# foollh/PicoPose

Hardware: AMD Instinct MI355X
Metric: image-crops/sec (224x224, 162 templates) (higher is better)
Workload: dtype f32 tensors; networks: f32 operands split into 2 f16 terms (22 bits) on f16 MFMA with f32 accumulate; stage-1 contraction: f16 MFMA operands, f32 accumulate, exact f32 re-evaluation of near-ties; PnP f64

## Files before the change

### picopose_amd/csrc/pp_attn.hip

```cpp

#include <hip/hip_runtime.h>
#include <stdint.h>
#include <stdlib.h>
#include "../../include/picopose_hip.h"
#include "pp_common.h"

namespace {

typedef float f32x16 __attribute__((ext_vector_type(16)));
typedef float f4 __attribute__((ext_vector_type(4)));

constexpr int HD = 64, KC = 32, KLD = 68;

constexpr int KTAIL_MAX = 4;
template <int WPB>
__global__ __launch_bounds__(64 * WPB) void attn_kernel(const float* __restrict__ qkv, int T, int heads, float scale,
                                                        float* __restrict__ out, _Float16* __restrict__ out_hl) {
    __shared__ __attribute__((aligned(16))) float Ks[KC * KLD];
    __shared__ __attribute__((aligned(16))) float Vs[KC * HD];
    const int tid = threadIdx.x, lane = tid & 63, w = tid >> 6, l31 = lane & 31, lh = lane >> 5;
    const int b = blockIdx.y / heads, h = blockIdx.y % heads;
    const int C3 = 3 * heads * HD;
    const float* base = qkv + (size_t)b * T * C3 + h * HD;
    const int q = blockIdx.x * (32 * WPB) + w * 32 + l31;
    const int qc = q < T ? q : T - 1;

    float qr[32];
    {
        const float* qp = base + (size_t)qc * C3 + 32 * lh;
#pragma unroll
        for (int p = 0; p < 32; p += 4) {
            const f4 v = *(const f4*)(qp + p);
            const float sc2 = scale * 1.44269504088896340736f;
            qr[p] = v.x * sc2; qr[p + 1] = v.y * sc2; qr[p + 2] = v.z * sc2; qr[p + 3] = v.w * sc2;
        }
    }
    f32x16 o0, o1;
#pragma unroll
    for (int e = 0; e < 16; ++e) o0[e] = o1[e] = 0.f;
    float mrun = -INFINITY, lrun = 0.f;

    const float* kp = base + heads * HD;
    const float* vp = base + 2 * heads * HD;
    const int ktail = (T % KC) <= KTAIL_MAX ? T % KC : 0;
    const int kend = T - ktail;
    for (int k0 = 0; k0 < kend; k0 += KC) {
        __syncthreads();
#pragma unroll
        for (int idx = tid; idx < KC * HD / 4; idx += 64 * WPB) {
            const int row = idx >> 4, c4 = (idx & 15) * 4;
            f4 kv = {0.f, 0.f, 0.f, 0.f}, vv = {0.f, 0.f, 0.f, 0.f};
            if (k0 + row < T) {
                kv = *(const f4*)(kp + (size_t)(k0 + row) * C3 + c4);
                vv = *(const f4*)(vp + (size_t)(k0 + row) * C3 + c4);
            }
            *(f4*)(Ks + row * KLD + c4) = kv;
            *(f4*)(Vs + row * HD + c4) = vv;
        }
        __syncthreads();
        f32x16 s;
#pragma unroll
        for (int e = 0; e < 16; ++e) s[e] = 0.f;
#pragma unroll
        for (int p4 = 0; p4 < 32; p4 += 4) {
            const f4 kf = *(const f4*)(Ks + l31 * KLD + 32 * lh + p4);
            s = __builtin_amdgcn_mfma_f32_32x32x2f32(kf.x, qr[p4], s, 0, 0, 0);
            s = __builtin_amdgcn_mfma_f32_32x32x2f32(kf.y, qr[p4 + 1], s, 0, 0, 0);
            s = __builtin_amdgcn_mfma_f32_32x32x2f32(kf.z, qr[p4 + 2], s, 0, 0, 0);
            s = __builtin_amdgcn_mfma_f32_32x32x2f32(kf.w, qr[p4 + 3], s, 0, 0, 0);
        }
        float mx = -INFINITY;
        if (k0 + KC <= T) {
#pragma unroll
            for (int e = 0; e < 16; ++e) mx = fmaxf(mx, s[e]);
        } else {
#pragma unroll
            for (int e = 0; e < 16; ++e) {
                const int key = k0 + (e & 3) + 8 * (e >> 2) + 4 * lh;
                s[e] = key < T ? s[e] : -INFINITY;
                mx = fmaxf(mx, s[e]);
            }
        }
        mx = fmaxf(mx, __shfl_xor(mx, 32));
        const float mnew = fmaxf(mrun, mx);
        const float alpha = __builtin_amdgcn_exp2f(mrun - mnew);
        float ls = 0.f;
#pragma unroll
        for (int e = 0; e < 16; ++e) {
            s[e] = __builtin_amdgcn_exp2f(s[e] - mnew);
            ls += s[e];
        }
        ls += __shfl_xor(ls, 32);
        lrun = lrun * alpha + ls;
        mrun = mnew;
#pragma unroll
        for (int e = 0; e < 16; ++e) {
            o0[e] *= alpha;
            o1[e] *= alpha;
        }
#pragma unroll
        for (int e = 0; e < 16; ++e) {
            const int key = (e & 3) + 8 * (e >> 2) + 4 * lh;
            const float v0 = Vs[key * HD + l31], v1 = Vs[key * HD + 32 + l31];
            o0 = __builtin_amdgcn_mfma_f32_32x32x2f32(v0, s[e], o0, 0, 0, 0);
            o1 = __builtin_amdgcn_mfma_f32_32x32x2f32(v1, s[e], o1, 0, 0, 0);
        }
    }
    for (int kx = kend; kx < T; ++kx) {
        const float* kr = kp + (size_t)kx * C3 + 32 * lh;
        float sp = 0.f;
#pragma unroll
        for (int p = 0; p < 32; p += 4) {
            const f4 kf = *(const f4*)(kr + p);
            sp = fmaf(kf.x, qr[p], sp);
            sp = fmaf(kf.y, qr[p + 1], sp);
            sp = fmaf(kf.z, qr[p + 2], sp);
            sp = fmaf(kf.w, qr[p + 3], sp);
        }
        const float sc = sp + __shfl_xor(sp, 32);
        const float mnew = fmaxf(mrun, sc);
        const float alpha = __builtin_amdgcn_exp2f(mrun - mnew);
        const float pk = __builtin_amdgcn_exp2f(sc - mnew);
        lrun = lrun * alpha + pk;
        mrun = mnew;
        const float* vr = vp + (size_t)kx * C3 + 4 * lh;
#pragma unroll
        for (int g = 0; g < 4; ++g) {
            const f4 v0 = *(const f4*)(vr + 8 * g), v1 = *(const f4*)(vr + 32 + 8 * g);
            o0[4 * g] = fmaf(v0.x, pk, o0[4 * g] * alpha);
            o0[4 * g + 1] = fmaf(v0.y, pk, o0[4 * g + 1] * alpha);
            o0[4 * g + 2] = fmaf(v0.z, pk, o0[4 * g + 2] * alpha);
            o0[4 * g + 3] = fmaf(v0.w, pk, o0[4 * g + 3] * alpha);
            o1[4 * g] = fmaf(v1.x, pk, o1[4 * g] * alpha);
            o1[4 * g + 1] = fmaf(v1.y, pk, o1[4 * g + 1] * alpha);
            o1[4 * g + 2] = fmaf(v1.z, pk, o1[4 * g + 2] * alpha);
            o1[4 * g + 3] = fmaf(v1.w, pk, o1[4 * g + 3] * alpha);
        }
    }
    if (q < T) {
        const float inv = 1.0f / lrun;
        const size_t obase = ((size_t)b * T + q) * (heads * HD) + h * HD;
#pragma unroll
        for (int e = 0; e < 16; ++e) {
            const int d = (e & 3) + 8 * (e >> 2) + 4 * lh;
            const float a0 = o0[e] * inv, a1 = o1[e] * inv;
            if (out) {
                out[obase + d] = a0;
                out[obase + 32 + d] = a1;
            }
            if (out_hl) {
                _Float16 hh, ll;
                pp_split_f16_chk(a0, hh, ll);
                out_hl[2 * obase + pp_hl_col(d, 0)] = hh;
                out_hl[2 * obase + pp_hl_col(d, 1)] = ll;
                pp_split_f16_chk(a1, hh, ll);
                out_hl[2 * obase + pp_hl_col(32 + d, 0)] = hh;
                out_hl[2 * obase + pp_hl_col(32 + d, 1)] = ll;
            }
        }
    }
}

typedef _Float16 h8 __attribute__((ext_vector_type(8)));
constexpr int KHLD = 72;
constexpr int VLD = 96;
typedef _Float16 h4 __attribute__((ext_vector_type(4)));
typedef __fp16 fp16x4_t __attribute__((__vector_size__(4 * sizeof(__fp16))));
constexpr int OLD = 68;
constexpr float P_SCALE = 1024.f;

__device__ __forceinline__ int vt_slot(int key) {
    const int s = key >> 4, r = key & 15;
    return s * 16 + ((r >> 2) & 1) * 8 + (r & 3) + 4 * (r >> 3);
}

template <int TERMS>
struct RingGeom {
    static constexpr int ROWH = 64 * TERMS;
    static constexpr int CPR = ROWH / 8;
    static constexpr int RPP = 64 / CPR;
    static constexpr int NPT = KC / RPP;
    static constexpr int STAGE_H = 2 * KC * ROWH;
};

template <bool HLIN, int TERMS = 2, int RING = 0, int WPB = 0>
__global__ __launch_bounds__(WPB > 4 ? 64 * WPB : 256) __attribute__((amdgpu_waves_per_eu(3, 3))) void attn_f16x3_kernel(const void* __restrict__ qkv_any, int T, int heads, float scale,
                                                         float* __restrict__ out, _Float16* __restrict__ out_hl,
                                                         float* __restrict__ lse, int ntx, int npairs) {
    static_assert(RING == 0 || (HLIN && WPB >= 1 && (WPB <= 4 || (WPB == 9 && RING == 8))), "the LDS-DMA ring copies operand rows");
    constexpr bool RESIDENT = RING == 8 && WPB == 9;
    using RG = RingGeom<TERMS>;
    extern __shared__ __attribute__((aligned(16))) unsigned char smem[];
    _Float16* Kh = (_Float16*)smem;
    _Float16* Kl = Kh + KC * KHLD;
    _Float16* Vh = Kl + KC * KHLD;
    _Float16* Vl = Vh + KC * VLD;
    const int tid = threadIdx.x, nthr = blockDim.x, lane = tid & 63, w = RING ? __builtin_amdgcn_readfirstlane(tid >> 6) : tid >> 6, l31 = lane & 31, lh = lane >> 5;
    const int xcd = blockIdx.x & 7, jj = blockIdx.x >> 3, bx = jj % ntx, pair = (jj / ntx) * 8 + xcd;
    if (pair >= npairs) return;
    const int b = pair / heads, h = pair % heads;
    const int C3 = 3 * heads * HD;
    const float* base = (const float*)qkv_any + (size_t)b * T * C3 + h * HD;
    const _Float16* hbase = (const _Float16*)qkv_any + ((size_t)b * T * C3 + h * HD) * TERMS;
    const int q = (bx * (nthr >> 6) + w) * 32 + l31;
    const int qc = q < T ? q : T - 1;

    h8 qh[4], ql[4];
    if (HLIN) {
        const _Float16* qp = hbase + (size_t)qc * C3 * TERMS;
#pragma unroll
        for (int s = 0; s < 4; ++s) {
            qh[s] = *(const h8*)(qp + TERMS * (16 * s + 8 * lh));
            if (TERMS == 2) ql[s] = *(const h8*)(qp + 2 * (16 * s + 8 * lh) + 8);
            else ql[s] = h8{0, 0, 0, 0, 0, 0, 0, 0};
        }
    } else {
        const float* qp = base + (size_t)qc * C3;
#pragma unroll
        for (int s = 0; s < 4; ++s) {
            const f4 a = *(const f4*)(qp + 16 * s + 8 * lh), c = *(const f4*)(qp + 16 * s + 8 * lh + 4);
#pragma unroll
            for (int i = 0; i < 4; ++i) {
                _Float16 hh, ll;
                pp_split_f16_chk(a[i], hh, ll);
                qh[s][i] = hh;
                ql[s][i] = ll;
                pp_split_f16_chk(c[i], hh, ll);
                qh[s][4 + i] = hh;
                ql[s][4 + i] = ll;
            }
        }
    }
    f32x16 o0, o1;
#pragma unroll
    for (int e = 0; e < 16; ++e) o0[e] = o1[e] = 0.f;
    float mrun = -INFINITY, lrun = 0.f;
    const float* kp = base + heads * HD;
    const float* vp = base + 2 * heads * HD;
    const float S_DESCALE = scale * 1.44269504088896340736f / (PP_A_SCALE * PP_A_SCALE);
    constexpr float O_RESCALE = 1.0f / PP_A_SCALE;
#define SOFTMAX_STEP(K0)                                                                                          \
    float mx = -INFINITY;                                                                                         \
    if ((K0) + KC > Tm) {        \
        _Pragma("unroll") for (int e = 0; e < 16; ++e) {                                                          \
            const int key = (K0) + (e & 3) + 8 * (e >> 2) + 4 * lh;                                               \
            sacc[e] = key < Tm ? sacc[e] : -INFINITY;                                                             \
        }                                                                                                         \
    }                                                                                                             \
    _Pragma("unroll") for (int e = 0; e < 16; ++e) mx = fmaxf(mx, sacc[e]);                                       \
    mx = fmaxf(mx, __shfl_xor(mx, 32));                                                                           \
    const float mnew = fmaxf(mrun, mx * S_DESCALE);                                                               \
    const float alpha = __builtin_amdgcn_exp2f(mrun - mnew);                                                      \
    const float shift = 10.0f - mnew;                                                                             \
    float ls = 0.f;                                                                                               \
    h8 ph[2], pl[2];                                                                                              \
    _Pragma("unroll") for (int e = 0; e < 16; ++e) {                                                              \
        const float x = __builtin_amdgcn_exp2f(fmaf(sacc[e], S_DESCALE, shift));              \
        ls += x;                                                                                                  \
        const _Float16 hh = (_Float16)x;                                                                          \
        ph[e >> 3][e & 7] = hh;                                                                                   \
        pl[e >> 3][e & 7] = (_Float16)(x - (float)hh);                                                            \
    }                                                                                                             \
    ls += __shfl_xor(ls, 32);                                                                                     \
    lrun = lrun * alpha + ls;                                                                                     \
    mrun = mnew;                                                                                                  \
    if (__builtin_amdgcn_ballot_w64(alpha != 1.0f) != 0) {                                                        \
        _Pragma("unroll") for (int e = 0; e < 16; ++e) {                                                          \
            o0[e] *= alpha;                                                                                       \
            o1[e] *= alpha;                                                                                       \
        }                                                                                                         \
    }

    constexpr int TAILMAX = 4;
    const int ntail = (T % KC) <= TAILMAX ? T % KC : 0, Tm = T - ntail;
    constexpr int NIT = HLIN ? 2 : 4;
    h8 pk[HLIN ? 2 * NIT : 1], pv[HLIN ? 2 * NIT : 1];
    f4 fk[HLIN ? 1 : NIT], fv[HLIN ? 1 : NIT];
    auto fetch = [&](int k0) __attribute__((always_inline)) {
#pragma unroll
        for (int it = 0; it < NIT; ++it) {
            const int idx = tid + it * nthr;
            if (HLIN) {
                const int row = idx >> 3, g = idx & 7;
                h8 z = {0, 0, 0, 0, 0, 0, 0, 0};
                pk[2 * it] = pk[2 * it + 1] = pv[2 * it] = pv[2 * it + 1] = z;
                if (idx < KC * (HD / 8) && k0 + row < Tm) {
                    const _Float16* kp2 = hbase + ((size_t)(k0 + row) * C3 + heads * HD + 8 * g) * TERMS;
                    const _Float16* vp2 = hbase + ((size_t)(k0 + row) * C3 + 2 * heads * HD + 8 * g) * TERMS;
                    pk[2 * it] = *(const h8*)kp2;
                    pv[2 * it] = *(const h8*)vp2;
                    if (TERMS == 2) {
                        pk[2 * it + 1] = *(const h8*)(kp2 + 8);
                        pv[2 * it + 1] = *(const h8*)(vp2 + 8);
                    }
                }
            } else {
                const int row = idx >> 4, c4 = (idx & 15) * 4;
                fk[it] = fv[it] = f4{0.f, 0.f, 0.f, 0.f};
                if (idx < KC * (HD / 4) && k0 + row < Tm) {
                    fk[it] = *(const f4*)(kp + (size_t)(k0 + row) * C3 + c4);
                    fv[it] = *(const f4*)(vp + (size_t)(k0 + row) * C3 + c4);
                }
            }
        }
    };
    auto commit = [&]() __attribute__((always_inline)) {
#pragma unroll
        for (int it = 0; it < NIT; ++it) {
            const int idx = tid + it * nthr;
            if (HLIN) {
                if (idx >= KC * (HD / 8)) continue;
                const int row = idx >> 3, g = idx & 7, slot = vt_slot(row);
                *(h8*)(Kh + row * KHLD + 8 * g) = pk[2 * it];
                *(h8*)(Vh + slot * VLD + 8 * g) = pv[2 * it];
                if (TERMS == 2) {
                    *(h8*)(Kl + row * KHLD + 8 * g) = pk[2 * it + 1];
                    *(h8*)(Vl + slot * VLD + 8 * g) = pv[2 * it + 1];
                }
            } else {
                if (idx >= KC * (HD / 4)) continue;
                const int row = idx >> 4, c4 = (idx & 15) * 4, slot = vt_slot(row);
                h4 khh, kll, vhh, vll;
#pragma unroll
                for (int i = 0; i < 4; ++i) {
                    _Float16 hh, ll;
                    pp_split_f16_chk(fk[it][i], hh, ll);
                    khh[i] = hh;
                    kll[i] = ll;
                    pp_split_f16_chk(fv[it][i], hh, ll);
                    vhh[i] = hh;
                    vll[i] = ll;
                }
                *(h4*)(Kh + row * KHLD + c4) = khh;
                *(h4*)(Kl + row * KHLD + c4) = kll;
                *(h4*)(Vh + slot * VLD + c4) = vhh;
                *(h4*)(Vl + slot * VLD + c4) = vll;
            }
        }
    };
    constexpr int NPW = RING ? (2 * RG::NPT + (WPB > 0 ? WPB : 1) - 1) / (WPB > 0 ? WPB : 1) : 1;
    unsigned poff[NPW];
    int prow[NPW];
    const __amdgpu_buffer_rsrc_t Hr = __builtin_amdgcn_make_buffer_rsrc(
        (void*)hbase, 0, RING ? (int)(((size_t)(T - 1) * C3 + 2 * heads * HD + HD) * 2 * TERMS) : 0, 0x00020000);
    if (RING) {
#pragma unroll
        for (int i = 0; i < NPW; ++i) {
            const int p = (w + (WPB > 0 ? WPB : 1) * i) % (2 * RG::NPT), isv = p / RG::NPT;
            const int rho = (p % RG::NPT) * RG::RPP + lane / RG::CPR, pos = lane % RG::CPR;
            int key, xk;
            if (isv) {
                const int r16 = rho & 15;
                key = (rho & 16) | (((r16 >> 2) & 1) << 3) | ((r16 >> 3) << 2) | (r16 & 3);
                xk = TERMS == 2 ? ((rho & 1) | (((rho >> 1) & 1) << 3)) : (((rho >> 1) & 1) << 2);
            } else {
                key = rho;
                xk = TERMS == 2 ? (rho & 15) : ((rho >> 1) & 7);
            }
            prow[i] = key;
            poff[i] = (unsigned)(((size_t)key * C3 + (size_t)(1 + isv) * heads * HD) * 2 * TERMS + (unsigned)((pos ^ xk) * 16));
        }
    }
    auto ring_pieces = [&](int k0, int stage, int i0, int i1) __attribute__((always_inline)) {
        _Float16* st = (_Float16*)smem + stage * RG::STAGE_H;
        const unsigned kbytes = (unsigned)((size_t)k0 * C3 * 2 * TERMS);
#pragma unroll
        for (int i = 0; i < NPW; ++i) {
            if (i < i0 || i >= i1) continue;
            const int p = (w + (WPB > 0 ? WPB : 1) * i) % (2 * RG::NPT);
            const unsigned off = (k0 + prow[i] < Tm) ? poff[i] + kbytes : 0xFFFFFFFFu;
            __builtin_amdgcn_raw_ptr_buffer_load_lds(Hr, (__attribute__((address_space(3))) void*)(st + p * 512), 16, off, 0, 0, 0);
        }
    };
    auto ring_issue = [&](int k0, int stage) __attribute__((always_inline)) { ring_pieces(k0, stage, 0, NPW); };
    auto ring_slot = [&](int k0, int stage, int g) __attribute__((always_inline)) {
        if ((g * NPW) / 6 != ((g + 1) * NPW) / 6) {
            __builtin_amdgcn_sched_barrier(0);
            ring_pieces(k0, stage, (g * NPW) / 6, ((g + 1) * NPW) / 6);
            __builtin_amdgcn_sched_barrier(0);
        }
    };
    if constexpr (RING > 0) {
        const int nch = (Tm + KC - 1) / KC;
#pragma unroll
        for (int c = 0; c < (RESIDENT ? RING : RING - 1); ++c) ring_issue(c * KC, c);
        int stage = 0, fill = RING - 1;
        const int kx = TERMS == 2 ? (l31 & 15) : ((l31 >> 1) & 7);
        for (int c = 0; c < nch; ++c) {
            const int k0 = c * KC;
            if constexpr (RESIDENT) {
                switch (c) {
                    case 0: asm volatile("s_waitcnt vmcnt(%0)" ::"n"(7 * NPW) : "memory"); break;
                    case 1: asm volatile("s_waitcnt vmcnt(%0)" ::"n"(6 * NPW) : "memory"); break;
                    case 2: asm volatile("s_waitcnt vmcnt(%0)" ::"n"(5 * NPW) : "memory"); break;
                    case 3: asm volatile("s_waitcnt vmcnt(%0)" ::"n"(4 * NPW) : "memory"); break;
                    case 4: asm volatile("s_waitcnt vmcnt(%0)" ::"n"(3 * NPW) : "memory"); break;
                    case 5: asm volatile("s_waitcnt vmcnt(%0)" ::"n"(2 * NPW) : "memory"); break;
                    case 6: asm volatile("s_waitcnt vmcnt(%0)" ::"n"(1 * NPW) : "memory"); break;
                    default: asm volatile("s_waitcnt vmcnt(0)" ::: "memory"); break;
                }
            } else {
                asm volatile("s_waitcnt vmcnt(%0)" ::"n"((RING - 2) * NPW) : "memory");
            }
            __syncthreads();
#ifndef PP_ATTN_SPREAD
            if constexpr (!RESIDENT) ring_issue(k0 + (RING - 1) * KC, fill);
#endif
            const int kn = k0 + (RING - 1) * KC;
            (void)kn;
            const _Float16* Kst = (const _Float16*)smem + stage * RG::STAGE_H;
            const _Float16* Vst = Kst + KC * RG::ROWH;
            f32x16 sacc;
#pragma unroll
            for (int e = 0; e < 16; ++e) sacc[e] = 0.f;
#pragma unroll
            for (int s = 0; s < 4; ++s) {
                const int ch = TERMS == 2 ? 2 * (2 * s + lh) : 2 * s + lh;
                const h8 kh = *(const h8*)(Kst + l31 * RG::ROWH + ((ch ^ kx) * 8));
                if (TERMS == 2) {
                    const h8 kl = *(const h8*)(Kst + l31 * RG::ROWH + (((ch + 1) ^ kx) * 8));
                    sacc = __builtin_amdgcn_mfma_f32_32x32x16_f16(kl, qh[s], sacc, 0, 0, 0);
                    sacc = __builtin_amdgcn_mfma_f32_32x32x16_f16(kh, ql[s], sacc, 0, 0, 0);
                }
                sacc = __builtin_amdgcn_mfma_f32_32x32x16_f16(kh, qh[s], sacc, 0, 0, 0);
#ifdef PP_ATTN_SPREAD
                ring_slot(kn, fill, s);
#endif
            }
            SOFTMAX_STEP(k0)
            auto vfrag = [&](int term, int s, int dhalf) __attribute__((always_inline)) -> h8 {
                const int col = 32 * dhalf + 16 * ((lane >> 4) & 1) + 4 * (lane & 3);
                const int row = 16 * s + 8 * lh + ((lane & 15) >> 2);
                const int ch = TERMS == 2 ? 2 * (col >> 3) + term : (col >> 3);
                auto at = [&](int r) __attribute__((always_inline)) -> const _Float16* {
                    const int xv = TERMS == 2 ? ((r & 1) | (((r >> 1) & 1) << 3)) : (((r >> 1) & 1) << 2);
                    return Vst + r * RG::ROWH + ((ch ^ xv) * 8) + (col & 7);
                };
                const fp16x4_t lo4 = __builtin_amdgcn_ds_read_tr16_b64_v4f16((__attribute__((address_space(3))) fp16x4_t*)at(row));
                const fp16x4_t hi4 = __builtin_amdgcn_ds_read_tr16_b64_v4f16((__attribute__((address_space(3))) fp16x4_t*)at(row + 4));
                h8 r;
#pragma unroll
                for (int e = 0; e < 4; ++e) {
                    r[e] = (_Float16)lo4[e];
                    r[4 + e] = (_Float16)hi4[e];
                }
                return r;
            };
#pragma unroll
            for (int s = 0; s < 2; ++s) {
                const h8 v0h = vfrag(0, s, 0), v1h = vfrag(0, s, 1);
                if (TERMS == 2) {
                    const h8 v0l = vfrag(1, s, 0), v1l = vfrag(1, s, 1);
                    o0 = __builtin_amdgcn_mfma_f32_32x32x16_f16(v0l, ph[s], o0, 0, 0, 0);
                    o0 = __builtin_amdgcn_mfma_f32_32x32x16_f16(v0h, pl[s], o0, 0, 0, 0);
                    o1 = __builtin_amdgcn_mfma_f32_32x32x16_f16(v1l, ph[s], o1, 0, 0, 0);
                    o1 = __builtin_amdgcn_mfma_f32_32x32x16_f16(v1h, pl[s], o1, 0, 0, 0);
                }
                o0 = __builtin_amdgcn_mfma_f32_32x32x16_f16(v0h, ph[s], o0, 0, 0, 0);
                o1 = __builtin_amdgcn_mfma_f32_32x32x16_f16(v1h, ph[s], o1, 0, 0, 0);
#ifdef PP_ATTN_SPREAD
                ring_slot(kn, fill, 4 + s);
#endif
            }
            fill = stage;
            stage = stage + 1 == RING ? 0 : stage + 1;
        }
        asm volatile("s_waitcnt vmcnt(0)" ::: "memory");
    } else {
    if (Tm > 0) fetch(0);
    for (int k0 = 0; k0 < Tm; k0 += KC) {
        __syncthreads();
        commit();
        __syncthreads();
        if (k0 + KC < Tm) fetch(k0 + KC);
        f32x16 sacc;
#pragma unroll
        for (int e = 0; e < 16; ++e) sacc[e] = 0.f;
#pragma unroll
        for (int s = 0; s < 4; ++s) {
            const h8 kh = *(const h8*)(Kh + l31 * KHLD + 16 * s + 8 * lh);
            if (TERMS == 2) {
                const h8 kl = *(const h8*)(Kl + l31 * KHLD + 16 * s + 8 * lh);
                sacc = __builtin_amdgcn_mfma_f32_32x32x16_f16(kl, qh[s], sacc, 0, 0, 0);
                sacc = __builtin_amdgcn_mfma_f32_32x32x16_f16(kh, ql[s], sacc, 0, 0, 0);
            }
            sacc = __builtin_amdgcn_mfma_f32_32x32x16_f16(kh, qh[s], sacc, 0, 0, 0);
        }
        SOFTMAX_STEP(k0)
        auto vfrag = [&](const _Float16* V, int s, int dhalf) __attribute__((always_inline)) -> h8 {
            const int col = 32 * dhalf + 16 * ((lane >> 4) & 1) + 4 * (lane & 3);
            const int row = 16 * s + 8 * lh + ((lane & 15) >> 2);
            const _Float16* p = V + row * VLD + col;
            const fp16x4_t lo4 = __builtin_amdgcn_ds_read_tr16_b64_v4f16((__attribute__((address_space(3))) fp16x4_t*)p);
            const fp16x4_t hi4 = __builtin_amdgcn_ds_read_tr16_b64_v4f16((__attribute__((address_space(3))) fp16x4_t*)(p + 4 * VLD));
            h8 r;
#pragma unroll
            for (int e = 0; e < 4; ++e) {
                r[e] = (_Float16)lo4[e];
                r[4 + e] = (_Float16)hi4[e];
            }
            return r;
        };
#pragma unroll
        for (int s = 0; s < 2; ++s) {
            const h8 v0h = vfrag(Vh, s, 0), v1h = vfrag(Vh, s, 1);
            if (TERMS == 2) {
                const h8 v0l = vfrag(Vl, s, 0), v1l = vfrag(Vl, s, 1);
                o0 = __builtin_amdgcn_mfma_f32_32x32x16_f16(v0l, ph[s], o0, 0, 0, 0);
                o0 = __builtin_amdgcn_mfma_f32_32x32x16_f16(v0h, pl[s], o0, 0, 0, 0);
                o1 = __builtin_amdgcn_mfma_f32_32x32x16_f16(v1l, ph[s], o1, 0, 0, 0);
                o1 = __builtin_amdgcn_mfma_f32_32x32x16_f16(v1h, pl[s], o1, 0, 0, 0);
            }
            o0 = __builtin_amdgcn_mfma_f32_32x32x16_f16(v0h, ph[s], o0, 0, 0, 0);
            o1 = __builtin_amdgcn_mfma_f32_32x32x16_f16(v1h, ph[s], o1, 0, 0, 0);
        }
    }
    }
    if (ntail > 0) {
        __syncthreads();
        float* tk = (float*)smem;
        float* tv = tk + TAILMAX * HD;
        for (int idx = tid; idx < ntail * HD; idx += nthr) {
            const int r = idx / HD, dd = idx - r * HD;
            float kf, vf;
            if (HLIN && TERMS == 1) {
                kf = (float)hbase[(size_t)(Tm + r) * C3 + heads * HD + dd];
                vf = (float)hbase[(size_t)(Tm + r) * C3 + 2 * heads * HD + dd];
            } else if (HLIN) {
                const _Float16* kp2 = hbase + ((size_t)(Tm + r) * C3 + heads * HD) * 2 + pp_hl_col(dd, 0);
                const _Float16* vp2 = hbase + ((size_t)(Tm + r) * C3 + 2 * heads * HD) * 2 + pp_hl_col(dd, 0);
                kf = (float)kp2[0] + (float)kp2[8];
                vf = (float)vp2[0] + (float)vp2[8];
            } else {
                _Float16 hh, ll;
                pp_split_f16_chk(kp[(size_t)(Tm + r) * C3 + dd], hh, ll);
                kf = (float)hh + (float)ll;
                pp_split_f16_chk(vp[(size_t)(Tm + r) * C3 + dd], hh, ll);
                vf = (float)hh + (float)ll;
            }
            tk[idx] = kf;
            tv[idx] = vf;
        }
        __syncthreads();
        for (int r = 0; r < ntail; ++r) {
            float dot = 0.f;
#pragma unroll
            for (int s4 = 0; s4 < 4; ++s4)
#pragma unroll
                for (int i = 0; i < 8; ++i)
                    dot = fmaf((float)qh[s4][i] + (float)ql[s4][i], tk[r * HD + 16 * s4 + 8 * lh + i], dot);
            dot += __shfl_xor(dot, 32);
            const float sv = dot * S_DESCALE;
            const float mnew = fmaxf(mrun, sv);
            const float alpha = __builtin_amdgcn_exp2f(mrun - mnew), pw = __builtin_amdgcn_exp2f(sv - mnew + 10.0f);
            lrun = lrun * alpha + pw;
            mrun = mnew;
#pragma unroll
            for (int e = 0; e < 16; ++e) {
                const int dd = (e & 3) + 8 * (e >> 2) + 4 * lh;
                o0[e] = fmaf(tv[r * HD + dd], pw, o0[e] * alpha);
                o1[e] = fmaf(tv[r * HD + 32 + dd], pw, o1[e] * alpha);
            }
        }
    }
    if (lse && q < T && lh == 0) lse[((size_t)b * heads + h) * T + q] = mrun + __builtin_amdgcn_logf(lrun) - 10.0f;
    __syncthreads();
    float* Os = (float*)smem + w * 32 * OLD;
    const float inv = O_RESCALE / lrun;
#pragma unroll
    for (int g = 0; g < 4; ++g) {
        f4 a, c;
#pragma unroll
        for (int i = 0; i < 4; ++i) {
            a[i] = o0[4 * g + i] * inv;
            c[i] = o1[4 * g + i] * inv;
        }
        *(f4*)(Os + l31 * OLD + 8 * g + 4 * lh) = a;
        *(f4*)(Os + l31 * OLD + 32 + 8 * g + 4 * lh) = c;
    }
    __builtin_amdgcn_s_waitcnt(0xc07f);
    const int qr = lane >> 1, half = lane & 1;
    const int qo = (bx * (nthr >> 6) + w) * 32 + qr;
    if (qo < T) {
        const size_t obase = ((size_t)b * T + qo) * (heads * HD) + h * HD + 32 * half;
        const float* src = Os + qr * OLD + 32 * half;
#pragma unroll
        for (int j = 0; j < 8; ++j) {
            const f4 v = *(const f4*)(src + 4 * j);
            if (out) *(f4*)(out + obase + 4 * j) = v;
            if (out_hl) {
                typedef _Float16 h4 __attribute__((ext_vector_type(4)));
                h4 hh, ll;
#pragma unroll
                for (int i = 0; i < 4; ++i) {
                    _Float16 a, c;
                    pp_split_f16_chk(v[i], a, c);
                    hh[i] = a;
                    ll[i] = c;
                }
                if (TERMS == 2) {
                    _Float16* hp = out_hl + 2 * obase + pp_hl_col(4 * j, 0);
                    *(h4*)hp = hh;
                    *(h4*)(hp + 8) = ll;
                } else {
                    *(h4*)(out_hl + obase + 4 * j) = hh;
                }
            }
        }
    }
}

}

PP_SAT_SETTER(pp_sat_set_attn)

extern "C" {

static int attention_launch(const void* qkv, bool hl_in, int B, int T, int heads, int head_dim, float scale, int prec, float* out,
                            void* out_hl, void* stream, int terms = 2, float* lse = nullptr) {
    if (!qkv || (!out && !out_hl) || B <= 0 || T <= 0 || heads <= 0 || (hl_in && prec != PP_PREC_F16X3)) return PP_EINVAL;
    if (terms == 1 && !hl_in) return PP_EINVAL;
    if (head_dim != HD || ((uintptr_t)qkv % 16) != 0) return PP_EINVAL;
    if (prec == PP_PREC_F16X3) {
        const int tiles = (T + 31) / 32;
        int wpb = 4, best = 1 << 30;
        for (int c = 4; c >= 2; --c) {
            const int waste = (tiles + c - 1) / c * c - tiles;
            if (waste < best) {
                best = waste;
                wpb = c;
            }
        }
        const size_t kv = (size_t)(2 * KC * KHLD + 2 * KC * VLD) * sizeof(_Float16), os = (size_t)wpb * 32 * OLD * sizeof(float);
        const int ntx = (tiles + wpb - 1) / wpb, npairs = B * heads;
        const dim3 grid((unsigned)(ntx * ((npairs + 7) / 8) * 8));
        const char* ring_s = getenv("PP_ATTN_RING");
        const int ring_env = ring_s ? atoi(ring_s) : 2;
        const size_t img_bytes = ((size_t)(T - 1) * 3 * heads * HD + 3 * heads * HD) * 2 * terms;
        const int tail_n = (T % KC) <= 4 ? T % KC : 0;
        if (hl_in && ring_env > 0 && ring_env != 1 && getenv("PP_ATTN_RESIDENT") != nullptr && lse == nullptr && img_bytes < 0x7FFFFFFFull && tiles == 9 &&
            T - tail_n == 8 * KC) {
            const dim3 grid9((unsigned)(((npairs + 7) / 8) * 8));
#define PP_ATTN_RES_LAUNCH(TERMS_)                                                                                                  \
    {                                                                                                                              \
        constexpr int lds_ = 8 * RingGeom<TERMS_>::STAGE_H * (int)sizeof(_Float16) > 9 * 32 * OLD * (int)sizeof(float)             \
                                 ? 8 * RingGeom<TERMS_>::STAGE_H * (int)sizeof(_Float16) : 9 * 32 * OLD * (int)sizeof(float);      \
        static signed char st_[PP_MAX_DEVICES];                                                                                    \
        signed char& ok_ = st_[pp_cur_device()];                                                                                   \
        if (ok_ == 0)                                                                                                              \
            ok_ = hipFuncSetAttribute((const void*)attn_f16x3_kernel<true, TERMS_, 8, 9>, hipFuncAttributeMaxDynamicSharedMemorySize, lds_) == hipSuccess ? 1 : -1; \
        if (ok_ < 0) return PP_ELAUNCH;                                                                                            \
        hipLaunchKernelGGL((attn_f16x3_kernel<true, TERMS_, 8, 9>), grid9, dim3(64 * 9), lds_, (hipStream_t)stream, qkv, T, heads, scale, out, \
                           (_Float16*)out_hl, lse, 1, npairs);                                                                     \
    }
            if (terms == 1) PP_ATTN_RES_LAUNCH(1) else PP_ATTN_RES_LAUNCH(2)
#undef PP_ATTN_RES_LAUNCH
            return pp_last_launch();
        }
        if (hl_in && (ring_env == 2 || ring_env == 3) && lse == nullptr && img_bytes < 0x7FFFFFFFull) {
            const size_t ring = (size_t)ring_env * RingGeom<2>::STAGE_H * sizeof(_Float16) * terms / 2;
            const size_t lds = ring > os ? ring : os;
#define PP_ATTN_RING_LAUNCH(TERMS_, S_, W_)                                                                                        \
    {                                                                                                                              \
        static signed char st_[PP_MAX_DEVICES];                                                                                    \
        signed char& ok_ = st_[pp_cur_device()];                                                                                   \
        if (ok_ == 0)                                                                                                              \
            ok_ = hipFuncSetAttribute((const void*)attn_f16x3_kernel<true, TERMS_, S_, W_>, hipFuncAttributeMaxDynamicSharedMemorySize, \
                                      (int)(S_ * RingGeom<TERMS_>::STAGE_H * sizeof(_Float16) > 4 * 32 * OLD * sizeof(float)               \
                                                ? S_ * RingGeom<TERMS_>::STAGE_H * sizeof(_Float16)                                  \
                                                : 4 * 32 * OLD * sizeof(float))) == hipSuccess ? 1 : -1;                            \
        if (ok_ < 0) return PP_ELAUNCH;                                                                                            \
        hipLaunchKernelGGL((attn_f16x3_kernel<true, TERMS_, S_, W_>), grid, dim3(64 * W_), lds, (hipStream_t)stream, qkv, T, heads, scale, out, \
                           (_Float16*)out_hl, lse, ntx, npairs);                                                                   \
    }
#define PP_ATTN_RING_W(TERMS_, S_)                                  \
    switch (wpb) {                                                  \
        case 2: PP_ATTN_RING_LAUNCH(TERMS_, S_, 2) break;           \
        case 3: PP_ATTN_RING_LAUNCH(TERMS_, S_, 3) break;           \
        default: PP_ATTN_RING_LAUNCH(TERMS_, S_, 4) break;          \
    }
            if (terms == 1) {
                if (ring_env == 2) PP_ATTN_RING_W(1, 2) else PP_ATTN_RING_W(1, 3)
            } else {
                if (ring_env == 2) PP_ATTN_RING_W(2, 2) else PP_ATTN_RING_W(2, 3)
            }
#undef PP_ATTN_RING_W
#undef PP_ATTN_RING_LAUNCH
            return pp_last_launch();
        }
        if (hl_in && terms == 1)
            hipLaunchKernelGGL((attn_f16x3_kernel<true, 1>), grid, dim3(64 * wpb), kv > os ? kv : os, (hipStream_t)stream, qkv, T, heads, scale, out,
                               (_Float16*)out_hl, lse, ntx, npairs);
        else if (hl_in)
            hipLaunchKernelGGL(attn_f16x3_kernel<true>, grid, dim3(64 * wpb), kv > os ? kv : os, (hipStream_t)stream, qkv, T, heads, scale, out,
                               (_Float16*)out_hl, lse, ntx, npairs);
        else
            hipLaunchKernelGGL(attn_f16x3_kernel<false>, grid, dim3(64 * wpb), kv > os ? kv : os, (hipStream_t)stream, qkv, T, heads, scale, out,
                               (_Float16*)out_hl, lse, ntx, npairs);
    } else {
        if (((T + 95) / 96) * 3 < ((T + 127) / 128) * 4)
            hipLaunchKernelGGL(attn_kernel<3>, dim3((T + 95) / 96, B * heads), dim3(192), 0, (hipStream_t)stream, (const float*)qkv, T, heads,
                               scale, out, (_Float16*)out_hl);
        else
            hipLaunchKernelGGL(attn_kernel<4>, dim3((T + 127) / 128, B * heads), dim3(256), 0, (hipStream_t)stream, (const float*)qkv, T, heads,
                               scale, out, (_Float16*)out_hl);
    }
    return pp_last_launch();
}

int pp_attention(const float* qkv, int B, int T, int heads, int head_dim, float scale, float* out, void* stream) {
    if (!out) return PP_EINVAL;
    return attention_launch(qkv, false, B, T, heads, head_dim, scale, PP_PREC_F32, out, nullptr, stream);
}

int pp_attention_split(const float* qkv, int B, int T, int heads, int head_dim, float scale, float* out, void* out_hl,
                       void* stream) {
    if (!out_hl) return PP_EINVAL;
    return attention_launch(qkv, false, B, T, heads, head_dim, scale, PP_PREC_F32, out, out_hl, stream);
}

int pp_attention_ex(const float* qkv, int B, int T, int heads, int head_dim, float scale, int prec, float* out, void* out_hl,
                    void* stream) {
    if (prec != PP_PREC_F32 && prec != PP_PREC_F16X3) return PP_EINVAL;
    return attention_launch(qkv, false, B, T, heads, head_dim, scale, prec, out, out_hl, stream);
}

int pp_attention_hl(const void* qkv_hl, int B, int T, int heads, int head_dim, float scale, float* out, void* out_hl,
                    void* stream) {
    if (((uintptr_t)qkv_hl % 16) != 0) return PP_EINVAL;
    return attention_launch(qkv_hl, true, B, T, heads, head_dim, scale, PP_PREC_F16X3, out, out_hl, stream);
}

int pp_attention_t(const void* qkv_operand, int terms, int B, int T, int heads, int head_dim, float scale, float* out, void* out_operand,
                   void* stream) {
    if (((uintptr_t)qkv_operand % 16) != 0 || (terms != 1 && terms != 2)) return PP_EINVAL;
    return attention_launch(qkv_operand, true, B, T, heads, head_dim, scale, PP_PREC_F16X3, out, out_operand, stream, terms);
}

int pp_attention_train(const float* qkv, int B, int T, int heads, int head_dim, float scale, float* out, float* lse2, void* stream) {
    if (!out || !lse2) return PP_EINVAL;
    return attention_launch(qkv, false, B, T, heads, head_dim, scale, PP_PREC_F16X3, out, nullptr, stream, 2, lse2);
}

}
```

Measured before the change: 521.1.

## Prefetch K/V LDS fragments with explicit waitcnt and coalesce ring-path epilogue stores

In the LDS-DMA ring attention path, K and V fragments are now loaded with inline-asm ds_read instructions from precomputed LDS offsets. The V transposed reads are issued before the softmax step, and fine-grained lgkmcnt waits let MFMAs start as soon as their operands arrive, overlapping LDS latency with compute. The DMA issue path drops the per-row bounds check on full chunks by passing the chunk offset as soffset. The epilogue writes 8 contiguous columns per lane with a single saturation flag, which is meant to improve store coalescing. Hand-written waitcnt counts are fragile and may be wrong if the compiler adds other LDS operations in between.

```diff
diff --git a/picopose_amd/csrc/pp_attn.hip b/picopose_amd/csrc/pp_attn.hip
--- a/picopose_amd/csrc/pp_attn.hip
+++ b/picopose_amd/csrc/pp_attn.hip
@@ -172,6 +172,10 @@
 __device__ __forceinline__ int vt_slot(int key) {
     const int s = key >> 4, r = key & 15;
     return s * 16 + ((r >> 2) & 1) * 8 + (r & 3) + 4 * (r >> 3);
+}
+
+__device__ __forceinline__ void lds_dma16(__amdgpu_buffer_rsrc_t rsrc, _Float16* dst, unsigned voff, int soff) {
+    __builtin_amdgcn_raw_ptr_buffer_load_lds(rsrc, (__attribute__((address_space(3))) void*)dst, 16, voff, soff, 0, 0);
 }
 
 template <int TERMS>
@@ -340,36 +344,42 @@
     };
     constexpr int NPW = RING ? (2 * RG::NPT + (WPB > 0 ? WPB : 1) - 1) / (WPB > 0 ? WPB : 1) : 1;
     unsigned poff[NPW];
-    int prow[NPW];
     const __amdgpu_buffer_rsrc_t Hr = __builtin_amdgcn_make_buffer_rsrc(
         (void*)hbase, 0, RING ? (int)(((size_t)(T - 1) * C3 + 2 * heads * HD + HD) * 2 * TERMS) : 0, 0x00020000);
+    auto piece_key = [&](int i) __attribute__((always_inline)) -> int {
+        const int p = (w + (WPB > 0 ? WPB : 1) * i) % (2 * RG::NPT), rho = (p % RG::NPT) * RG::RPP + lane / RG::CPR;
+        if (p / RG::NPT == 0) return rho;
+        const int r16 = rho & 15;
+        return (rho & 16) | (((r16 >> 2) & 1) << 3) | ((r16 >> 3) << 2) | (r16 & 3);
+    };
     if (RING) {
 #pragma unroll
         for (int i = 0; i < NPW; ++i) {
             const int p = (w + (WPB > 0 ? WPB : 1) * i) % (2 * RG::NPT), isv = p / RG::NPT;
             const int rho = (p % RG::NPT) * RG::RPP + lane / RG::CPR, pos = lane % RG::CPR;
-            int key, xk;
-            if (isv) {
-                const int r16 = rho & 15;
-                key = (rho & 16) | (((r16 >> 2) & 1) << 3) | ((r16 >> 3) << 2) | (r16 & 3);
-                xk = TERMS == 2 ? ((rho & 1) | (((rho >> 1) & 1) << 3)) : (((rho >> 1) & 1) << 2);
-            } else {
-                key = rho;
-                xk = TERMS == 2 ? (rho & 15) : ((rho >> 1) & 7);
-            }
-            prow[i] = key;
-            poff[i] = (unsigned)(((size_t)key * C3 + (size_t)(1 + isv) * heads * HD) * 2 * TERMS + (unsigned)((pos ^ xk) * 16));
+            int xk;
+            if (isv) xk = TERMS == 2 ? ((rho & 1) | (((rho >> 1) & 1) << 3)) : (((rho >> 1) & 1) << 2);
+            else xk = TERMS == 2 ? (rho & 15) : ((rho >> 1) & 7);
+            poff[i] = (unsigned)(((size_t)piece_key(i) * C3 + (size_t)(1 + isv) * heads * HD) * 2 * TERMS + (unsigned)((pos ^ xk) * 16));
         }
     }
     auto ring_pieces = [&](int k0, int stage, int i0, int i1) __attribute__((always_inline)) {
         _Float16* st = (_Float16*)smem + stage * RG::STAGE_H;
         const unsigned kbytes = (unsigned)((size_t)k0 * C3 * 2 * TERMS);
-#pragma unroll
-        for (int i = 0; i < NPW; ++i) {
-            if (i < i0 || i >= i1) continue;
-            const int p = (w + (WPB > 0 ? WPB : 1) * i) % (2 * RG::NPT);
-            const unsigned off = (k0 + prow[i] < Tm) ? poff[i] + kbytes : 0xFFFFFFFFu;
-            __builtin_amdgcn_raw_ptr_buffer_load_lds(Hr, (__attribute__((address_space(3))) void*)(st + p * 512), 16, off, 0, 0, 0);
+        if (NPW <= 6 && k0 + KC <= Tm) {
+#pragma unroll
+            for (int i = 0; i < NPW; ++i) {
+                if (i < i0 || i >= i1) continue;
+                const int p = (w + (WPB > 0 ? WPB : 1) * i) % (2 * RG::NPT);
+                lds_dma16(Hr, st + p * 512, poff[i], (int)kbytes);
+            }
+        } else {
+#pragma unroll
+            for (int i = 0; i < NPW; ++i) {
+                if (i < i0 || i >= i1) continue;
+                const int p = (w + (WPB > 0 ? WPB : 1) * i) % (2 * RG::NPT);
+                lds_dma16(Hr, st + p * 512, (k0 + piece_key(i) < Tm) ? poff[i] + kbytes : 0xFFFFFFFFu, 0);
+            }
         }
     };
     auto ring_issue = [&](int k0, int stage) __attribute__((always_inline)) { ring_pieces(k0, stage, 0, NPW); };
@@ -386,6 +396,41 @@
         for (int c = 0; c < (RESIDENT ? RING : RING - 1); ++c) ring_issue(c * KC, c);
         int stage = 0, fill = RING - 1;
         const int kx = TERMS == 2 ? (l31 & 15) : ((l31 >> 1) & 7);
+        const unsigned lds0 = (unsigned)(size_t)(__attribute__((address_space(3))) unsigned char*)smem;
+        unsigned voff[2 * TERMS];
+        {
+            const int r0 = 8 * lh + ((lane & 15) >> 2);
+            const int xv = TERMS == 2 ? ((r0 & 1) | (((r0 >> 1) & 1) << 3)) : (((r0 >> 1) & 1) << 2);
+#pragma unroll
+            for (int f = 0; f < 2 * TERMS; ++f) {
+                const int col = 32 * (f & 1) + 16 * ((lane >> 4) & 1) + 4 * (lane & 3);
+                const int ch = TERMS == 2 ? 2 * (col >> 3) + (f >> 1) : (col >> 3);
+                voff[f] = lds0 + 2u * (unsigned)(KC * RG::ROWH + r0 * RG::ROWH + ((ch ^ xv) * 8) + (col & 7));
+            }
+        }
+        h4 vq[2][2 * TERMS][2];
+#define PP_V_READ(S, F, G) \
+    asm volatile("ds_read_b64_tr_b16 %0, %1 offset:%2" : "=v"(vq[S][F][G]) : "v"(va[F]), "n"(((S) * 16 + (G) * 4) * RG::ROWH * 2) : "memory")
+#define PP_V_READS(S)                                                  \
+    _Pragma("unroll") for (int f = 0; f < 2 * TERMS; ++f) {            \
+        PP_V_READ(S, f, 0);                                            \
+        PP_V_READ(S, f, 1);                                            \
+    }
+#define PP_V_WAIT(S, N)                                                                                                            \
+    if constexpr (TERMS == 2)                                                                                                      \
+        asm volatile("s_waitcnt lgkmcnt(%[n])" : "+v"(vq[S][0][0]), "+v"(vq[S][0][1]), "+v"(vq[S][1][0]), "+v"(vq[S][1][1]),       \
+                     "+v"(vq[S][2][0]), "+v"(vq[S][2][1]), "+v"(vq[S][3][0]), "+v"(vq[S][3][1]) : [n] "n"(N) : "memory");          \
+    else                                                                                                                           \
+        asm volatile("s_waitcnt lgkmcnt(%[n])" : "+v"(vq[S][0][0]), "+v"(vq[S][0][1]), "+v"(vq[S][1][0]), "+v"(vq[S][1][1])        \
+                     : [n] "n"(N) : "memory");
+        unsigned koff[4][TERMS];
+#pragma unroll
+        for (int s = 0; s < 4; ++s)
+#pragma unroll
+            for (int t = 0; t < TERMS; ++t) {
+                const int ch = TERMS == 2 ? 2 * (2 * s + lh) + t : 2 * s + lh;
+                koff[s][t] = lds0 + 2u * (unsigned)(l31 * RG::ROWH + ((ch ^ kx) * 8));
+            }
         for (int c = 0; c < nch; ++c) {
             const int k0 = c * KC;
             if constexpr (RESIDENT) {
@@ -408,17 +453,39 @@
 #endif
             const int kn = k0 + (RING - 1) * KC;
             (void)kn;
-            const _Float16* Kst = (const _Float16*)smem + stage * RG::STAGE_H;
-            const _Float16* Vst = Kst + KC * RG::ROWH;
+            const unsigned stage_b = (unsigned)(stage * RG::STAGE_H * 2);
+            unsigned va[2 * TERMS];
+#pragma unroll
+            for (int f = 0; f < 2 * TERMS; ++f) va[f] = voff[f] + stage_b;
             f32x16 sacc;
 #pragma unroll
             for (int e = 0; e < 16; ++e) sacc[e] = 0.f;
+            h8 kq[4][TERMS];
+#pragma unroll
+            for (int s = 0; s < 4; ++s)
+#pragma unroll
+                for (int t = 0; t < TERMS; ++t)
+                    asm volatile("ds_read_b128 %0, %1" : "=v"(kq[s][t]) : "v"(koff[s][t] + stage_b) : "memory");
 #pragma unroll
             for (int s = 0; s < 4; ++s) {
-                const int ch = TERMS == 2 ? 2 * (2 * s + lh) : 2 * s + lh;
-                const h8 kh = *(const h8*)(Kst + l31 * RG::ROWH + ((ch ^ kx) * 8));
+                if constexpr (TERMS == 2) {
+                    switch (s) {
+                        case 0: asm volatile("s_waitcnt lgkmcnt(6)" : "+v"(kq[0][0]), "+v"(kq[0][1]) :: "memory"); break;
+                        case 1: asm volatile("s_waitcnt lgkmcnt(4)" : "+v"(kq[1][0]), "+v"(kq[1][1]) :: "memory"); break;
+                        case 2: asm volatile("s_waitcnt lgkmcnt(2)" : "+v"(kq[2][0]), "+v"(kq[2][1]) :: "memory"); break;
+                        default: asm volatile("s_waitcnt lgkmcnt(0)" : "+v"(kq[3][0]), "+v"(kq[3][1]) :: "memory"); break;
+                    }
+                } else {
+                    switch (s) {
+                        case 0: asm volatile("s_waitcnt lgkmcnt(3)" : "+v"(kq[0][0]) :: "memory"); break;
+                        case 1: asm volatile("s_waitcnt lgkmcnt(2)" : "+v"(kq[1][0]) :: "memory"); break;
+                        case 2: asm volatile("s_waitcnt lgkmcnt(1)" : "+v"(kq[2][0]) :: "memory"); break;
+                        default: asm volatile("s_waitcnt lgkmcnt(0)" : "+v"(kq[3][0]) :: "memory"); break;
+                    }
+                }
+                const h8 kh = kq[s][0];
                 if (TERMS == 2) {
-                    const h8 kl = *(const h8*)(Kst + l31 * RG::ROWH + (((ch + 1) ^ kx) * 8));
+                    const h8 kl = kq[s][TERMS - 1];
                     sacc = __builtin_amdgcn_mfma_f32_32x32x16_f16(kl, qh[s], sacc, 0, 0, 0);
                     sacc = __builtin_amdgcn_mfma_f32_32x32x16_f16(kh, ql[s], sacc, 0, 0, 0);
                 }
@@ -427,30 +494,18 @@
                 ring_slot(kn, fill, s);
 #endif
             }
+            PP_V_READS(0)
+            PP_V_READS(1)
             SOFTMAX_STEP(k0)
-            auto vfrag = [&](int term, int s, int dhalf) __attribute__((always_inline)) -> h8 {
-                const int col = 32 * dhalf + 16 * ((lane >> 4) & 1) + 4 * (lane & 3);
-                const int row = 16 * s + 8 * lh + ((lane & 15) >> 2);
-                const int ch = TERMS == 2 ? 2 * (col >> 3) + term : (col >> 3);
-                auto at = [&](int r) __attribute__((always_inline)) -> const _Float16* {
-                    const int xv = TERMS == 2 ? ((r & 1) | (((r >> 1) & 1) << 3)) : (((r >> 1) & 1) << 2);
-                    return Vst + r * RG::ROWH + ((ch ^ xv) * 8) + (col & 7);
+#pragma unroll
+            for (int s = 0; s < 2; ++s) {
+                if (s == 0) { PP_V_WAIT(0, 4 * TERMS) } else { PP_V_WAIT(1, 0) }
+                auto vfrag = [&](int f) __attribute__((always_inline)) -> h8 {
+                    return __builtin_shufflevector(vq[s][f][0], vq[s][f][1], 0, 1, 2, 3, 4, 5, 6, 7);
                 };
-                const fp16x4_t lo4 = __builtin_amdgcn_ds_read_tr16_b64_v4f16((__attribute__((address_space(3))) fp16x4_t*)at(row));
-                const fp16x4_t hi4 = __builtin_amdgcn_ds_read_tr16_b64_v4f16((__attribute__((address_space(3))) fp16x4_t*)at(row + 4));
-                h8 r;
-#pragma unroll
-                for (int e = 0; e < 4; ++e) {
-                    r[e] = (_Float16)lo4[e];
-                    r[4 + e] = (_Float16)hi4[e];
-                }
-                return r;
-            };
-#pragma unroll
-            for (int s = 0; s < 2; ++s) {
-                const h8 v0h = vfrag(0, s, 0), v1h = vfrag(0, s, 1);
+                const h8 v0h = vfrag(0), v1h = vfrag(1);
                 if (TERMS == 2) {
-                    const h8 v0l = vfrag(1, s, 0), v1l = vfrag(1, s, 1);
+                    const h8 v0l = vfrag(2 * (TERMS - 1)), v1l = vfrag(2 * (TERMS - 1) + 1);
                     o0 = __builtin_amdgcn_mfma_f32_32x32x16_f16(v0l, ph[s], o0, 0, 0, 0);
                     o0 = __builtin_amdgcn_mfma_f32_32x32x16_f16(v0h, pl[s], o0, 0, 0, 0);
                     o1 = __builtin_amdgcn_mfma_f32_32x32x16_f16(v1l, ph[s], o1, 0, 0, 0);
@@ -465,6 +520,9 @@
             fill = stage;
             stage = stage + 1 == RING ? 0 : stage + 1;
         }
+#undef PP_V_READ
+#undef PP_V_READS
+#undef PP_V_WAIT
         asm volatile("s_waitcnt vmcnt(0)" ::: "memory");
     } else {
     if (Tm > 0) fetch(0);
@@ -579,6 +637,45 @@
         *(f4*)(Os + l31 * OLD + 32 + 8 * g + 4 * lh) = c;
     }
     __builtin_amdgcn_s_waitcnt(0xc07f);
+    if constexpr (RING > 0) {
+        const int cg = lane & 7;
+        bool sat = false;
+#pragma unroll
+        for (int t = 0; t < 4; ++t) {
+            const int r = 8 * t + (lane >> 3), qo = (bx * (nthr >> 6) + w) * 32 + r;
+            const f4 va = *(const f4*)(Os + r * OLD + 8 * cg), vb = *(const f4*)(Os + r * OLD + 8 * cg + 4);
+            if (qo < T) {
+                const size_t obase = ((size_t)b * T + qo) * (heads * HD) + h * HD + 8 * cg;
+                if (out) {
+                    *(f4*)(out + obase) = va;
+                    *(f4*)(out + obase + 4) = vb;
+                }
+                if (out_hl) {
+                    h8 hh, ll;
+#pragma unroll
+                    for (int i = 0; i < 4; ++i) {
+                        _Float16 a, c;
+                        sat |= !(fabsf(va[i]) * PP_A_SCALE < 65504.f) | !(fabsf(vb[i]) * PP_A_SCALE < 65504.f);
+                        pp_split_f16(va[i], a, c);
+                        hh[i] = a;
+                        ll[i] = c;
+                        pp_split_f16(vb[i], a, c);
+                        hh[4 + i] = a;
+                        ll[4 + i] = c;
+                    }
+                    if (TERMS == 2) {
+                        _Float16* hp = out_hl + 2 * obase;
+                        *(h8*)hp = hh;
+                        *(h8*)(hp + 8) = ll;
+                    } else {
+                        *(h8*)(out_hl + obase) = hh;
+                    }
+                }
+            }
+        }
+        pp_sat_flag(sat);
+        return;
+    }
     const int qr = lane >> 1, half = lane & 1;
     const int qo = (bx * (nthr >> 6) + w) * 32 + qr;
     if (qo < T) {
```

New measurement: 524.9, median of 6. No clear change (+0.7%).
